# DigITs-AIML/MMNN_STS

Hardware: AMD Instinct MI355X
Metric: training volumes/sec/GPU (128^3 T1+T2+preop, batch 2) at 1/2/4/8 MI355X (higher is better)
Workload: dtype f32; 1 GPU; configs[2] --images --preop --survival --blend: MultiModalModel(DenseNet121-3D(in=2), MLP(32), blend) fwd + GradientBlender Cox loss + bwd + grad all-reduce + SGD-Nesterov/OneCycle step, dropout 0.2; micro_batch=2, global_batch=2, tabular=32, parallelism=dp1, allreduce=none

## Files before the change

mmnn_sts_amd/csrc/densenet.hip:

```cpp
#include "densenet.hpp"

#include <string.h>

#include <algorithm>

#include "fprop.hpp"
#include "stem.hpp"
#include "wgrad.hpp"

namespace mmnn {

constexpr size_t KZ_PART_BYTES = (size_t)512 * 4 * 1024 * sizeof(float);
constexpr unsigned KZ_CNT_ENTRIES = 4096;

namespace {
struct Panel { const float* p; unsigned bytes; };
struct LayerBind {
  BnFwd bn1, bn2;
  BnBwd gr_new, gr_t1;
  StatPtr dg1, dg2, s_x;
  View x, g;
  View x_new, g_new;
  View t1, dz2;
};
// ... 193 lines not shown
  return concat_site(p, b, lo.cin, lo.n1w, lo.n1b, lo.r1m, lo.r1v, p.o_dg_n1[b][l]);
}
static NormSite norm2(const Plan& p, int b, int l) {
  const LayerOff& lo = p.layers[b][l];
  return {p.o_st_t1[b][l], p.o_dg_n2[b][l], p.o_dg_n2[b][l], p.mid, 0, p.mid, p.nrep_b[b], lo.n2w, lo.n2b, lo.r2m, lo.r2v, (double)p.N * p.Vb[b]};
}
static NormSite transition(const Plan& p, int b) {
  const TransOff& t = p.trans[b];
  return concat_site(p, b, t.cin, t.nw, t.nb, t.rm, t.rv, p.o_dg_tr[b]);
}
static NormSite norm5(const Plan& p) {
  const int b = p.cfg.nblocks - 1;
  return concat_site(p, b, p.ctot_b[b], p.p_n5w, p.p_n5b, p.r_n5m, p.r_n5v, p.o_dg_n5);
}

static StatPtr statptr(char* ws, size_t o, int C, int off, int nrep) {
  StatPtr s; memset(&s, 0, sizeof(s));
  s.sum = reinterpret_cast<double*>(ws + o); s.sq = s.sum + (long)NREP * C;
  s.stride = C; s.off = off; s.nrep = nrep;
  return s;
}
static StatPtr stats(char* ws, const NormSite& s, int first = 0, int training = 1) {
  StatPtr st = statptr(ws, s.o_st, s.stride, s.off + first, s.nrep);
  if (!training) st.sum = nullptr;
  return st;
}
static StatPtr sums(char* ws, const NormSite& s, int first = 0) { return statptr(ws, s.o_s, s.stride, s.off + first, s.nrep); }
static StatPtr dgsums(char* ws, const NormSite& s) { return statptr(ws, s.o_dg, s.C, 0, s.nrep); }
static BnFwd bnfwd(const Plan& p, char* ws, const float* params, float* run, const NormSite& s, int training) {
  BnFwd f; memset(&f, 0, sizeof(f));
  f.st = stats(ws, s);
  f.rmean = run + s.rm; f.rvar = run + s.rv; f.gamma = params + s.w; f.beta = params + s.b;
  f.inv_count = 1.0 / s.count; f.eps = p.cfg.eps; f.training = training;
  return f;
}
static BnBwd bnbwd(const Plan& p, char* ws, const float* params, const NormSite& s, int first = 0) {
  BnBwd g; memset(&g, 0, sizeof(g));
  g.st = stats(ws, s, first); g.s = sums(ws, s, first);
  g.gamma = s.o_s == s.o_dg ? params + s.w : nullptr;
  g.inv_count = 1.0 / s.count; g.eps = p.cfg.eps;
  return g;
}

static float* fptr(char* ws, size_t o) { return reinterpret_cast<float*>(ws + o); }
static View concat(const Plan& p, char* ws, int b, int coff = 0) { return {fptr(ws, p.o_x[b]), (long)p.ctot_b[b] * p.Vb[b], coff}; }
static View concat_grad(const Plan& p, char* ws, int b, int coff = 0) { return {fptr(ws, p.o_g[b]), (long)p.ctot_b[b] * p.Vb[b], coff}; }
static View t1(const Plan& p, char* ws, int b, int l) { return {fptr(ws, p.o_t1[b][l]), (long)p.mid * p.Vb[b], 0}; }
static View dz2(const Plan& p, char* ws, int b, int l) { return {fptr(ws, p.o_dz2[b]) + (long)l * p.N * p.mid * p.Vb[b], (long)p.mid * p.Vb[b], 0}; }
static View pooled(const Plan& p, char* ws, int b) { return {fptr(ws, p.o_ap[b]), (long)p.ctot_b[b] * p.Vb[b + 1], 0}; }
static View pooled_grad(const Plan& p, char* ws, int b) { return {fptr(ws, p.o_dap), (long)p.ctot_b[b] * p.Vb[b + 1], 0}; }

static void set_in0(FpropArgs& a, View v) { a.in0 = v.p; a.in0_ns = v.ns; a.in0_coff = v.coff; }
static void set_in1(FpropArgs& a, View v) { a.in1 = v.p; a.in1_ns = v.ns; a.in1_coff = v.coff; }
static void set_out(FpropArgs& a, View v) { a.out = v.p; a.out_ns = v.ns; a.out_coff = v.coff; }
static void set_ex(FpropArgs& a, View v) { a.ex = v.p; a.ex_ns = v.ns; a.ex_coff = v.coff; }
static void set_g0(WgradArgs& a, View v) { a.g0 = v.p; a.g0_ns = v.ns; a.g0_coff = v.coff; }
static void set_g1(WgradArgs& a, View v) { a.g1 = v.p; a.g1_ns = v.ns; a.g1_coff = v.coff; }
static void set_x(WgradArgs& a, View v) { a.x = v.p; a.x_ns = v.ns; a.x_coff = v.coff; }

static Panel conv1_panel(const Plan& p, char* ws, int b, int l) { return {fptr(ws, p.o_pk_c1[b][l]), (unsigned)(sizeof(float) * conv1_elems(p, p.layers[b][l].cin))}; }
static Panel trans_panel(const Plan& p, char* ws, int b) { return {fptr(ws, p.o_pk_tr[b]), (unsigned)(sizeof(float) * trans_elems(p.trans[b]))}; }
static Panel conv1_weights(const Plan& p, const float* params, int b, int l) { return {params + p.layers[b][l].c1, (unsigned)(sizeof(float) * conv1_elems(p, p.layers[b][l].cin))}; }
static Panel conv2_panel(const Plan& p, char* ws, int b, int l, bool bwd, bool fp32 = false) {
  const size_t o3 = (bwd ? p.o_pk_c2b3 : p.o_pk_c2f3)[b][l];
  if (o3 && !fp32) return {fptr(ws, o3), (unsigned)conv2_split_bytes(p)};
  return {fptr(ws, (bwd ? p.o_pk_c2b : p.o_pk_c2f)[b][l]), (unsigned)(sizeof(float) * conv2_elems(p))};
}
static void set_conv2_weights(FpropArgs& a, const Plan& p, char* ws, int b, int l, bool bwd) {
  const Panel w = conv2_panel(p, ws, b, l, bwd, true), w3 = conv2_panel(p, ws, b, l, bwd);
  a.w = w.p;
  if (w3.p != w.p) { a.w3 = w3.p; a.x3 = ws + p.o_x3; a.x3_bytes = p.x3_bytes; }
}
static void prefetch(FpropArgs& a, Panel w) { a.pf_ptr = w.p; a.pf_bytes = w.bytes; }

static unsigned long long* trace_slot(const Plan& p) {
  return (p.trace_base && p.trace_seq < p.trace_slots) ? p.trace_base + (size_t)(p.trace_seq++) * 64 * 16 : nullptr;
}

static FpropArgs block_args(const Plan& p, char* ws, int b) {
  FpropArgs a; memset(&a, 0, sizeof(a));
  a.N = p.N; a.D = p.Db[b]; a.H = p.Hb[b]; a.W = p.Wb[b]; a.nrep = p.nrep_b[b];
  a.kz_part = p.no_kz ? nullptr : fptr(ws, p.o_kz_part); a.kz_cnt = reinterpret_cast<unsigned*>(ws + p.o_kz_cnt);
  a.kz_part_bytes = KZ_PART_BYTES; a.kz_cnt_entries = KZ_CNT_ENTRIES;
  a.trace = trace_slot(p);
  return a;
}
static void wgrad_shape(WgradArgs& w, const Plan& p, int b) {
  memset(&w, 0, sizeof(w));
  w.N = p.N; w.D = p.Db[b]; w.H = p.Hb[b]; w.W = p.Wb[b];
}

static bool build_tables(Plan& p, const float* params, float* run, char* ws) {
  if (p.tab_params == params && p.tab_run == run && p.tab_ws == ws) return false;
  char* hj = static_cast<char*>(p.host_jobs);
  RunStatJob* rj = reinterpret_cast<RunStatJob*>(hj);
  PackJob* pj = reinterpret_cast<PackJob*>(hj + (p.o_jobs_pack - p.o_jobs_run));
  GradJob* gj = reinterpret_cast<GradJob*>(hj + (p.o_jobs_grad - p.o_jobs_run));
  const NetCfg& c = p.cfg;
  const int nb = c.nblocks;
  int ir = 0, ip = 0, ig = 0;
  p.max_pack = 0; p.max_grad = 0;
  auto pack_job = [&](long src, size_t dst, int kind, int M, int C, long count) {
    PackJob& j = pj[ip++]; memset(&j, 0, sizeof(j));
    j.src = params + src; j.dst = fptr(ws, dst); j.kind = kind; j.M = M; j.C = C; j.count = count;
    p.max_pack = std::max(p.max_pack, count);
  };
  auto grad_job = [&](int kind, const void* src, long stride, int ns, int M, int C, long dst, long count) {
    GradJob& j = gj[ig++]; memset(&j, 0, sizeof(j));
    j.kind = kind; j.src = src; j.stride = stride; j.nsplit = ns; j.M = M; j.C = C; j.dst_off = dst; j.count = count;
    p.max_grad = std::max(p.max_grad, count);
  };
  auto grad_slab = [&](int kind, size_t o, int ns, int M, int C, long dst, long count) {
    grad_job(kind, ws + o, kind == 2 ? (long)C * M * 352 : count, ns, M, C, dst, count);
  };
  auto site_jobs = [&](const NormSite& s) {
    const StatPtr st = stats(ws, s), dg = dgsums(ws, s);
    RunStatJob& j = rj[ir++]; memset(&j, 0, sizeof(j));
    j.sum = st.sum; j.sq = st.sq; j.stride = s.stride; j.off = s.off; j.C = s.C;
    j.rmean = run ? run + s.rm : nullptr; j.rvar = run ? run + s.rv : nullptr; j.count = s.count;
    grad_job(3, dg.sq, s.C, 0, 0, s.C, s.w, s.C);
    grad_job(3, dg.sum, s.C, 0, 0, s.C, s.b, s.C);
  };
  pack_job(p.p_conv0, p.o_pk_conv0, (c.in_channels % 2 == 0) ? 3 : 4, c.init_features, c.in_channels, (long)7 * stem_krows(c.in_channels) * 64);
  grad_slab(2, p.o_sl_conv0, p.ns_conv0, c.init_features, c.in_channels, p.p_conv0, (long)c.init_features * c.in_channels * 343);
  site_jobs(norm0(p));
  for (int b = 0; b < nb; ++b) {
    p.gj_begin[b] = ig;
    const long max_before = p.max_grad;
    p.max_grad = 0;
    for (int l = 0; l < c.block_layers[b]; ++l) {
      const LayerOff& lo = p.layers[b][l];
      pack_job(lo.c1, p.o_pk_c1[b][l], 0, p.mid, lo.cin, conv1_elems(p, lo.cin));
      pack_job(lo.c2, p.o_pk_c2f[b][l], 1, c.growth, p.mid, conv2_elems(p));
      pack_job(lo.c2, p.o_pk_c2b[b][l], 2, c.growth, p.mid, conv2_elems(p));
      if (p.o_pk_c2f3[b][l]) pack_job(lo.c2, p.o_pk_c2f3[b][l], 5, c.growth, p.mid, (long)27 * (p.mid / 8) * c.growth);
      if (p.o_pk_c2b3[b][l]) pack_job(lo.c2, p.o_pk_c2b3[b][l], 6, c.growth, p.mid, (long)27 * (c.growth / 8) * p.mid);
      site_jobs(norm1(p, b, l));
      grad_slab(0, p.o_sl_c1[b][l], p.ns_c1[b][l], p.mid, lo.cin, lo.c1, conv1_elems(p, lo.cin));
      site_jobs(norm2(p, b, l));
      grad_slab(1, p.o_sl_c2[b][l], p.ns_c2[b][l], c.growth, p.mid, lo.c2, conv2_elems(p));
    }
    if (b != nb - 1) {
      const TransOff& t = p.trans[b];
      pack_job(t.cw, p.o_pk_tr[b], 0, t.cout, t.cin, trans_elems(t));
      site_jobs(transition(p, b));
      grad_slab(0, p.o_sl_tr[b], p.ns_tr[b], t.cout, t.cin, t.cw, trans_elems(t));
    } else {
      site_jobs(norm5(p));
    }
    p.gj_max[b] = p.max_grad;
    p.max_grad = std::max(p.max_grad, max_before);
  }
  p.gj_begin[nb] = ig;
  p.n_run_jobs = ir; p.n_pack_jobs = ip; p.n_grad_jobs = ig;
  p.tab_params = params; p.tab_run = run; p.tab_ws = ws;
  return true;
}

namespace {
struct ScopedTimer {
  Plan& p; hipStream_t s; bool on;
  ScopedTimer(Plan& p_, int kind, int block, hipStream_t s_) : p(p_), s(s_), on(false) {
    if (!((p.timer_mask >> kind) & 1u) || (p.timer_block >= 0 && p.timer_block != block)) return;
    if (p.timer_used + 2 > p.timer_ev.size()) {
      if (p.timer_ev.size() >= 16384) return;
      hipEvent_t a, b;
      if (hipEventCreate(&a) != hipSuccess || hipEventCreate(&b) != hipSuccess) return;
      p.timer_ev.push_back(a); p.timer_ev.push_back(b);
      p.timer_tag.push_back(0);
    }
    p.timer_tag[p.timer_used / 2] = kind * MAX_BLOCKS + (block >= 0 && block < MAX_BLOCKS ? block : 0);
    on = hipEventRecord(p.timer_ev[p.timer_used], s) == hipSuccess;
  }
  ~ScopedTimer() {
    if (!on) return;
    (void)hipEventRecord(p.timer_ev[p.timer_used + 1], s);
    p.timer_used += 2;
  }
};
}

int plan_set_timer(Plan& p, int kind, int block) {
  MMNN_REQUIRE(kind >= -1 && kind < T_COUNT, "set_timer: unknown kernel class %d", kind);
  p.timer_mask = kind < 0 ? ~1u : (kind == T_NONE ? 0u : 1u << kind);
  p.timer_block = block; p.timer_used = 0;
  for (int k = 0; k < T_COUNT * MAX_BLOCKS; ++k) { p.timer_ms[k] = 0.0; p.timer_count[k] = 0; }
  return 0;
}

int plan_read_timer(Plan& p, int kind, int block, double* total_ms, long* count) {
  MMNN_REQUIRE(kind >= T_NONE && kind < T_COUNT && block < MAX_BLOCKS, "read_timer: unknown kernel class %d / block %d", kind, block);
  for (size_t i = 0; i + 1 < p.timer_used; i += 2) {
    MMNN_HIP(hipEventSynchronize(p.timer_ev[i + 1]));
    float ms = 0.f;
    MMNN_HIP(hipEventElapsedTime(&ms, p.timer_ev[i], p.timer_ev[i + 1]));
    const int k = p.timer_tag[i / 2];
    p.timer_ms[k] += ms; p.timer_count[k] += 1;
  }
  p.timer_used = 0;
  double ms = 0.0; long n = 0;
  for (int k = 1; k < T_COUNT; ++k)
    for (int b = 0; b < MAX_BLOCKS; ++b)
      if ((kind == T_NONE || kind == k) && (block < 0 || block == b)) { ms += p.timer_ms[k * MAX_BLOCKS + b]; n += p.timer_count[k * MAX_BLOCKS + b]; }
  if (total_ms) *total_ms = ms;
  if (count) *count = n;
  return 0;
}

int plan_set_option(Plan& p, const char* name, long value) {
  const std::string s(name ? name : "");
  if (s == "single_stream") return 0;
  if (s == "trace_buffer") { p.trace_base = reinterpret_cast<unsigned long long*>(value); p.trace_seq = 0; return 0; }
  if (s == "trace_slots") { p.trace_slots = (int)value; return 0; }
  if (s == "params_version") { p.params_version = value; return 0; }
  if (s == "no_kz") { p.no_kz = value != 0; return 0; }
  set_error("set_option: unknown option '%s'", s.c_str());
  return 1;
}
static DropCfg dropcfg(const Plan& p, uint64_t seed, int layer, int training) {
  DropCfg d; memset(&d, 0, sizeof(d));
  d.seed = seed; d.layer = layer; d.p = training ? p.cfg.dropout_p : 0.f;
  return d;
}

int plan_forward(Plan& p, const float* params, float* run, const float* x, char* ws, float* out, int training, uint64_t seed,
                 hipStream_t stream) {
  MMNN_REQUIRE(params && run && x && ws && out, "forward: null buffer");
  MMNN_REQUIRE(((uintptr_t)ws & 255) == 0 && ((uintptr_t)params & 15) == 0 && ((uintptr_t)x & 15) == 0, "forward: buffers must be 256/16-byte aligned");
  const NetCfg& c = p.cfg;
  const int nb = c.nblocks, N = p.N;
  if (!p.host_jobs) {
    MMNN_HIP(hipHostMalloc(&p.host_jobs, p.host_jobs_bytes, hipHostMallocDefault));
    memset(p.host_jobs, 0, p.host_jobs_bytes);
  }
  if (p.tab_params != params || p.tab_run != run || p.tab_ws != ws) {
    if (p.tab_ws != nullptr) MMNN_HIP(hipStreamSynchronize(stream));
    build_tables(p, params, run, ws);
    MMNN_HIP(hipMemcpyAsync(ws + p.o_jobs_run, p.host_jobs, p.host_jobs_bytes, hipMemcpyHostToDevice, stream));
  }
  p.trace_seq = 0;
  if (training) MMNN_HIP(hipMemsetAsync(ws + p.o_fstat, 0, p.fstat_bytes, stream));
  MMNN_HIP(hipMemsetAsync(ws + p.o_kz_cnt, 0, KZ_CNT_ENTRIES * sizeof(unsigned), stream));
  int rc = 0;
  if (p.params_version == 0 || p.params_version != p.packed_version || p.packed_params != params || p.packed_ws != ws) {
    rc = launch_pack(reinterpret_cast<const PackJob*>(ws + p.o_jobs_pack), p.n_pack_jobs, p.max_pack, stream);
    if (rc) return rc;
    p.packed_version = p.params_version; p.packed_params = params; p.packed_ws = ws;
    ++p.pack_launches;
  }

  {
    const NormSite n0 = norm0(p);
    StemConvArgs a; memset(&a, 0, sizeof(a));
    a.N = N; a.Cin = c.in_channels; a.D = p.D; a.H = p.H; a.W = p.W; a.Do = p.D0; a.Ho = p.H0; a.Wo = p.W0; a.M = c.init_features;
    a.x = x; a.wp = fptr(ws, p.o_pk_conv0); a.out = fptr(ws, p.o_conv0);
    a.st_out = stats(ws, n0, 0, training);
    { ScopedTimer t(p, T_STEM_CONV, -1, stream); rc = launch_stem_conv(a, stream); }
    if (rc) return rc;
    const View X = concat(p, ws, 0);
    StemPoolArgs q; memset(&q, 0, sizeof(q));
    q.N = N; q.C = c.init_features; q.Di = p.D0; q.Hi = p.H0; q.Wi = p.W0; q.Do = p.Db[0]; q.Ho = p.Hb[0]; q.Wo = p.Wb[0];
    q.x = fptr(ws, p.o_conv0);
    q.bn = bnfwd(p, ws, params, run, n0, training);
    q.out = X.p; q.out_ns = X.ns;
    q.idx = reinterpret_cast<unsigned char*>(ws + p.o_idx);
    q.st_out = stats(ws, norm1(p, 0, 0), 0, training);
    if ((rc = launch_stem_pool(q, stream))) return rc;
  }
  int layer_id = 0;
  for (int b = 0; b < nb; ++b) {
    const View X = concat(p, ws, b);
    for (int l = 0; l < c.block_layers[b]; ++l, ++layer_id) {
      const NormSite n1 = norm1(p, b, l), n2 = norm2(p, b, l);
      FpropArgs a = block_args(p, ws, b);
      a.Cin = n1.C; a.M = p.mid;
      set_in0(a, X);
      a.bn_in = bnfwd(p, ws, params, run, n1, training);
      a.w = conv1_panel(p, ws, b, l).p; a.w_ld = p.mid;
      set_out(a, t1(p, ws, b, l));
      a.st_out = stats(ws, n2, 0, training);
      prefetch(a, conv2_panel(p, ws, b, l, false));
      { ScopedTimer t(p, T_CONV1_FWD, b, stream); rc = launch_fprop(a, 1, PRO_BNRELU, EPI_STORE_STATS, stream); }
      if (rc) return rc;
      FpropArgs e = block_args(p, ws, b);
      e.Cin = p.mid; e.M = c.growth;
      set_in0(e, t1(p, ws, b, l));
      e.bn_in = bnfwd(p, ws, params, run, n2, training);
      set_conv2_weights(e, p, ws, b, l, false); e.w_ld = c.growth;
      set_out(e, concat(p, ws, b, n1.C));
      e.drop_out = dropcfg(p, seed, layer_id, training);
      e.st_out = stats(ws, n1, n1.C, training);
      if (l + 1 < c.block_layers[b]) prefetch(e, conv1_panel(p, ws, b, l + 1));
      else if (b != nb - 1) prefetch(e, trans_panel(p, ws, b));
      { ScopedTimer t(p, T_CONV2_FWD, b, stream); rc = launch_fprop(e, 27, PRO_BNRELU, EPI_STORE_STATS, stream); }
      if (rc) return rc;
    }
    if (b != nb - 1) {
      const NormSite tr = transition(p, b);
// ... 186 lines not shown
      if ((rc = launch_wgrad1(w, PRO_NONE, stream))) return rc;
      FpropArgs d = block_args(p, ws, b);
      d.nrep = 0;
      d.Cin = t.cout; d.M = t.cin;
      set_in0(d, G); set_in1(d, X); d.gr_in = gr;
      d.w = params + t.cw; d.w_ld = t.cin;
      set_out(d, pooled_grad(p, ws, pb));
      if ((rc = launch_fprop(d, 1, PRO_GRAD, EPI_STORE, stream))) return rc;
      if ((rc = launch_consumer_bwd(consumer_bwd_args(p, params, run, ws, transition(p, pb), pb, 1, pooled_grad(p, ws, pb).p), stream))) return rc;
    } else {
      const NormSite n0 = norm0(p);
      const StatPtr dg = dgsums(ws, n0);
      StemPoolBwdArgs q; memset(&q, 0, sizeof(q));
      q.N = N; q.C = c.init_features; q.Di = p.D0; q.Hi = p.H0; q.Wi = p.W0; q.Do = p.Db[0]; q.Ho = p.Hb[0]; q.Wo = p.Wb[0];
      q.x = fptr(ws, p.o_conv0);
      q.bn = bnfwd(p, ws, params, run, n0, 1);
      q.g = G.p; q.g_ns = G.ns; q.xp = X.p; q.xp_ns = X.ns;
      q.gr = gr;
      q.idx = reinterpret_cast<const unsigned char*>(ws + p.o_idx);
      q.dz = fptr(ws, p.o_dz0);
      q.dbeta = dg.sum; q.dgamma = dg.sq;
      if ((rc = launch_stem_pool_bwd(q, stream))) return rc;
      StemWgradArgs w; memset(&w, 0, sizeof(w));
      w.N = N; w.Cin = c.in_channels; w.D = p.D; w.H = p.H; w.W = p.W; w.Do = p.D0; w.Ho = p.H0; w.Wo = p.W0; w.M = c.init_features;
      w.x = x; w.dz = fptr(ws, p.o_dz0); w.y = fptr(ws, p.o_conv0);
      w.gr = bnbwd(p, ws, params, n0);
      w.slab = fptr(ws, p.o_sl_conv0); w.slab_stride = (long)c.in_channels * c.init_features * 352; w.nsplit = p.ns_conv0;
      { ScopedTimer t(p, T_STEM_WGRAD, -1, stream); rc = launch_stem_wgrad(w, stream); }
      if (rc) return rc;
    }
  }
  const long stem_count = (long)c.init_features * c.in_channels * 343;
  const GradJob* jobs = reinterpret_cast<const GradJob*>(ws + p.o_jobs_grad);
  const int j0 = lo == 0 ? 0 : p.gj_begin[lo], j1 = p.gj_begin[hi + 1];
  long jmax = lo == 0 ? stem_count : 0;
  for (int b = lo; b <= hi; ++b) jmax = std::max(jmax, p.gj_max[b]);
  return launch_finalize(jobs + j0, j1 - j0, jmax, grad_params, accumulate, stream);
}

int plan_relu_mask(Plan& p, const float* params, char* ws, int kind, int b, int l, unsigned char* out, hipStream_t stream) {
  MMNN_REQUIRE(p.tab_ws == ws && p.tab_params == params, "relu_mask: must follow a training forward on the same buffers");
  const NetCfg& c = p.cfg;
  MMNN_REQUIRE(kind == 0 || (b >= 0 && b < c.nblocks), "relu_mask: bad block %d", b);
  MMNN_REQUIRE(kind != 3 || b < c.nblocks - 1, "relu_mask: block %d has no transition", b);
  MMNN_REQUIRE(kind == 0 || kind == 3 || (l >= 0 && l < c.block_layers[b] && (kind == 1 || kind == 2)), "relu_mask: bad site (%d,%d,%d)", kind, b, l);
  const NormSite s = kind == 0 ? norm0(p) : kind == 1 ? norm1(p, b, l) : kind == 2 ? norm2(p, b, l) : transition(p, b);
  const int V = kind == 0 ? p.D0 * p.H0 * p.W0 : p.Vb[b];
  const View X = kind == 0 ? View{fptr(ws, p.o_conv0), (long)s.C * V, 0} : kind == 2 ? t1(p, ws, b, l) : concat(p, ws, b);
  MaskArgs a; memset(&a, 0, sizeof(a));
  a.out = out; a.N = p.N; a.C = s.C; a.V = V; a.x = X.p; a.x_ns = X.ns;
  a.bn = bnfwd(p, ws, params, p.tab_run, s, 1);
  return launch_relu_mask(a, stream);
}

long plan_ws_offset(const Plan& p, const char* name, int i, int j) {
  const std::string s(name);
  const int nb = p.cfg.nblocks;
  auto okb = [&](int b) { return b >= 0 && b < nb; };
  auto okl = [&](int b, int l) { return okb(b) && l >= 0 && l < p.cfg.block_layers[b]; };
  if (s == "conv0") return (long)p.o_conv0;
  if (s == "idx") return (long)p.o_idx;
  if (s == "dz0") return (long)p.o_dz0;
  if (s == "dz2" && okl(i, j)) return (long)(p.o_dz2[i] + (size_t)j * p.N * p.mid * p.Vb[i] * sizeof(float));
  if (s == "dap") return (long)p.o_dap;
  if (s == "x" && okb(i)) return (long)p.o_x[i];
  if (s == "g" && okb(i)) return (long)p.o_g[i];
  if (s == "ap" && okb(i) && i < nb - 1) return (long)p.o_ap[i];
  if (s == "t1" && okl(i, j)) return (long)p.o_t1[i][j];
  if (s == "st_conv0") return (long)p.o_st_conv0;
  if (s == "st_x" && okb(i)) return (long)p.o_st_x[i];
  if (s == "st_t1" && okl(i, j)) return (long)p.o_st_t1[i][j];
  if (s == "s_x" && okb(i)) return (long)p.o_s_x[i];
  if (s == "pk_c1" && okl(i, j)) return (long)p.o_pk_c1[i][j];
  if (s == "pk_c2f" && okl(i, j)) return (long)p.o_pk_c2f[i][j];
  if (s == "pk_c2b" && okl(i, j)) return (long)p.o_pk_c2b[i][j];
  if (s == "pk_c2f3" && okl(i, j)) return p.o_pk_c2f3[i][j] ? (long)p.o_pk_c2f3[i][j] : -1;
  if (s == "pk_c2b3" && okl(i, j)) return p.o_pk_c2b3[i][j] ? (long)p.o_pk_c2b3[i][j] : -1;
  if (s == "x3") return p.x3_bytes ? (long)p.o_x3 : -1;
  if (s == "#x3_bytes") return (long)p.x3_bytes;
  if (s == "pk_conv0") return (long)p.o_pk_conv0;
  if (s == "#pack_launches") return p.pack_launches;
  if (s == "#ns_c2" && okl(i, j)) return p.ns_c2[i][j];
  if (s == "#ns_c1" && okl(i, j)) return p.ns_c1[i][j];
  return -1;
}

}
```

mmnn_sts_amd/csrc/densenet.hpp:

```cpp
#pragma once
#include <string>
#include <vector>

#include "common.hpp"
#include "elementwise.hpp"

namespace mmnn {

constexpr int MAX_BLOCKS = 8;

struct NetCfg {
  int in_channels, init_features, growth, bn_size, nblocks;
  int block_layers[MAX_BLOCKS];
  float eps, momentum, dropout_p;
};

struct LayerOff {
  long n1w, n1b, c1, n2w, n2b, c2;
  long r1m, r1v, r2m, r2v;
  int cin;
};
struct TransOff { long nw, nb, cw; long rm, rv; int cin, cout; };

struct NormSite {
  size_t o_st;
  size_t o_s;
  size_t o_dg;
  int stride, off, C, nrep;
  long w, b, rm, rv;
  double count;
};
struct View { float* p; long ns; int coff; };

struct Plan {
  NetCfg cfg;
  int N, D, H, W;
  int D0, H0, W0;
  int Db[MAX_BLOCKS], Hb[MAX_BLOCKS], Wb[MAX_BLOCKS], Vb[MAX_BLOCKS];
  int cin_b[MAX_BLOCKS], ctot_b[MAX_BLOCKS];
  int nrep_b[MAX_BLOCKS];
  int mid;
  long p_conv0, p_n0w, p_n0b, r_n0m, r_n0v, p_n5w, p_n5b, r_n5m, r_n5v;
  std::vector<std::vector<LayerOff>> layers;
  std::vector<TransOff> trans;
  long n_params, n_runstats;
  int n_bn;
  size_t ws_bytes;
  size_t o_conv0, o_idx, o_x[MAX_BLOCKS], o_g[MAX_BLOCKS], o_ap[MAX_BLOCKS], o_dz2[MAX_BLOCKS], o_dap, o_dz0;
  std::vector<std::vector<size_t>> o_t1;
  size_t o_fstat, fstat_bytes, o_bstat, bstat_bytes;
  size_t o_st_conv0, o_st_x[MAX_BLOCKS];
  std::vector<std::vector<size_t>> o_st_t1;
  size_t o_s_x[MAX_BLOCKS];
  size_t o_dg_n0, o_dg_n5;
  std::vector<std::vector<size_t>> o_dg_n1, o_dg_n2;
  std::vector<size_t> o_dg_tr;
  size_t o_pk_conv0;
  std::vector<std::vector<size_t>> o_pk_c1, o_pk_c2f, o_pk_c2b;
  std::vector<std::vector<size_t>> o_pk_c2f3, o_pk_c2b3;
  size_t o_x3 = 0, x3_bytes = 0;
  std::vector<size_t> o_pk_tr;
  size_t o_sl_conv0; int ns_conv0;
  std::vector<std::vector<size_t>> o_sl_c1, o_sl_c2;
  std::vector<std::vector<int>> ns_c1, ns_c2;
  std::vector<size_t> o_sl_tr; std::vector<int> ns_tr;
  size_t o_kz_part, o_kz_cnt;
  size_t o_jobs_run, o_jobs_pack, o_jobs_grad;
  int n_layers = 0;
  size_t o_wg_table = 0;
  void* wg_pinned = nullptr; std::vector<char> wg_shadow; bool wg_uploaded = false;
  void* host_jobs = nullptr; size_t host_jobs_bytes = 0;
  const float* tab_params = nullptr; float* tab_run = nullptr; char* tab_ws = nullptr;
  int n_run_jobs = 0, n_pack_jobs = 0, n_grad_jobs = 0; long max_pack = 0, max_grad = 0;
  int gj_begin[MAX_BLOCKS + 1] = {0};
  long gj_max[MAX_BLOCKS] = {0};
  unsigned timer_mask = 0; int timer_block = -1;
  std::vector<hipEvent_t> timer_ev;
  std::vector<int> timer_tag;
  size_t timer_used = 0;
  double timer_ms[16 * MAX_BLOCKS] = {0}; long timer_count[16 * MAX_BLOCKS] = {0};
  long params_version = 0, packed_version = 0; const float* packed_params = nullptr; const char* packed_ws = nullptr;
  long pack_launches = 0;
  long long* nbt = nullptr; int nbt_count = 0;
  bool no_kz = false;
  int bwd_next = -1;
  unsigned long long* trace_base = nullptr; mutable int trace_seq = 0; int trace_slots = 0;
};

enum TimerKind { T_NONE = 0, T_CONV2_FWD = 1, T_CONV2_DGRAD = 2, T_CONV2_WGRAD = 3, T_CONV1_FWD = 4, T_CONV1_DGRAD = 5,
                 T_CONV1_WGRAD = 6, T_STEM_CONV = 7, T_STEM_WGRAD = 8, T_BLOCK_FWD = 9, T_COUNT = 10 };
int plan_set_timer(Plan& p, int kind, int block);
int plan_read_timer(Plan& p, int kind, int block, double* total_ms, long* count);
int plan_set_option(Plan& p, const char* name, long value);

int plan_build(Plan& p, const NetCfg& cfg, int N, int D, int H, int W);
void plan_free(Plan& p);
int plan_forward(Plan& p, const float* params, float* runstats, const float* x, char* ws, float* out, int training,
                 uint64_t seed, hipStream_t stream);
int plan_backward(Plan& p, const float* params, const float* x, char* ws, const float* grad_out, float* grad_params,
                  int accumulate, uint64_t seed, hipStream_t stream);
int plan_backward_range(Plan& p, const float* params, const float* x, char* ws, const float* grad_out, float* grad_params,
                        int accumulate, uint64_t seed, int hi, int lo, hipStream_t stream);
int plan_block_param_range(const Plan& p, int block, long* begin, long* end);
long plan_ws_offset(const Plan& p, const char* name, int i, int j);
int plan_relu_mask(Plan& p, const float* params, char* ws, int kind, int b, int l, unsigned char* out, hipStream_t stream);

}
```

mmnn_sts_amd/csrc/fprop.hip:

```cpp
#include <stdlib.h>

#include "fprop.hpp"

namespace mmnn {

template <int TAPS, int PRO, int EPI>
int dispatch(const FpropArgs& a, hipStream_t s);
extern template int dispatch<1, PRO_BNRELU, EPI_STORE_STATS>(const FpropArgs&, hipStream_t);
extern template int dispatch<1, PRO_NONE, EPI_STORE_STATS>(const FpropArgs&, hipStream_t);
extern template int dispatch<1, PRO_GRAD, EPI_MASK_ACCUM>(const FpropArgs&, hipStream_t);
extern template int dispatch<1, PRO_GRAD, EPI_STORE>(const FpropArgs&, hipStream_t);
extern template int dispatch<27, PRO_BNRELU, EPI_STORE_STATS>(const FpropArgs&, hipStream_t);
extern template int dispatch<27, PRO_GRAD, EPI_MASK_STORE>(const FpropArgs&, hipStream_t);

bool conv3_fwd_bf16x3_eligible(const FpropArgs& a);
int launch_conv3_fwd_bf16x3(const FpropArgs& a, hipStream_t stream);
bool conv3_dgrad_bf16x3_eligible(const FpropArgs& a);
int launch_conv3_dgrad_bf16x3(const FpropArgs& a, hipStream_t stream);

int launch_fprop(const FpropArgs& a, int taps, int pro, int epi, hipStream_t stream) {
  MMNN_REQUIRE(a.N > 0 && a.D > 0 && a.H > 0 && a.W > 0 && a.Cin > 0 && a.M > 0, "fprop: non-positive extent");
  MMNN_REQUIRE((long)a.D * a.H * a.W < (1l << 30), "fprop: volume too large for 32-bit voxel indices");
  MMNN_REQUIRE(a.in0 && a.w && a.out && a.w_ld >= a.M, "fprop: null operand or w_ld < M");
  MMNN_REQUIRE((long)(a.M + 128) * a.D * a.H * a.W < (1l << 31), "fprop: output rows x volume too large for 32-bit element offsets");
  MMNN_REQUIRE(pro != PRO_GRAD || a.in1, "fprop: PRO_GRAD needs the normalised tensor (in1)");
  MMNN_REQUIRE((epi != EPI_MASK_STORE && epi != EPI_MASK_ACCUM) || (a.ex && a.dgamma && a.dbeta), "fprop: mask epilogue operands missing");
  if (taps == 27 && pro == PRO_BNRELU && epi == EPI_STORE_STATS && conv3_fwd_bf16x3_eligible(a)) return launch_conv3_fwd_bf16x3(a, stream);
  if (taps == 27 && pro == PRO_GRAD && epi == EPI_MASK_STORE && conv3_dgrad_bf16x3_eligible(a)) return launch_conv3_dgrad_bf16x3(a, stream);
#define MMNN_CASE(T, P, E) \
  if (taps == T && pro == P && epi == E) return dispatch<T, P, E>(a, stream);
  MMNN_CASE(1, PRO_BNRELU, EPI_STORE_STATS)
  MMNN_CASE(1, PRO_NONE, EPI_STORE_STATS)
  MMNN_CASE(1, PRO_GRAD, EPI_MASK_ACCUM)
  MMNN_CASE(1, PRO_GRAD, EPI_STORE)
  MMNN_CASE(27, PRO_BNRELU, EPI_STORE_STATS)
  MMNN_CASE(27, PRO_GRAD, EPI_MASK_STORE)
#undef MMNN_CASE
  set_error("fprop: unsupported (taps=%d, pro=%d, epi=%d)", taps, pro, epi);
  return 1;
}

}
```

mmnn_sts_amd/csrc/fprop.hpp:

```cpp
#pragma once
#include "common.hpp"

namespace mmnn {

#if !defined(MMNN_KZ_FENCED)
#if defined(__gfx950__) || !defined(__HIP_DEVICE_COMPILE__)
#define MMNN_KZ_FENCED 0
#else
#define MMNN_KZ_FENCED 1
#endif
#endif

enum Pro { PRO_NONE = 0, PRO_BNRELU = 1, PRO_GRAD = 2 };
enum Epi { EPI_STORE = 0, EPI_STORE_STATS = 1, EPI_MASK_STORE = 2, EPI_MASK_ACCUM = 3 };

struct FpropArgs {
  int N, D, H, W;
  int Cin, M;
  const float* in0; long in0_ns; int in0_coff;
  const float* in1; long in1_ns; int in1_coff;
  BnFwd bn_in;
  BnBwd gr_in;
  DropCfg drop_in;
  const float* w; int w_ld;
  float* out; long out_ns; int out_coff;
  DropCfg drop_out;
  StatPtr st_out;
  const float* ex; long ex_ns; int ex_coff;
  BnFwd ebn;
  double* dgamma; double* dbeta;
  StatPtr s_acc;
  int nrep;
  float* kz_part; unsigned* kz_cnt;
  size_t kz_part_bytes; unsigned kz_cnt_entries;
  const float* pf_ptr; unsigned pf_bytes;
  const void* w3; void* x3; size_t x3_bytes;
  unsigned mg_w, mg_h, mg_d;
  unsigned long long* trace;
};

int launch_fprop(const FpropArgs& a, int taps, int pro, int epi, hipStream_t stream);
bool conv3_fwd_bf16x3_eligible(const FpropArgs& a);
bool conv3_dgrad_bf16x3_eligible(const FpropArgs& a);
size_t conv3_bf16x3_plane_bytes(const FpropArgs& a);

#if defined(__HIPCC__)

template <int TAPS, int PRO, int EPI, int WM, int WN, int KS, int MT, int NT, int KC, int TD, int TH, int TW, bool SPEC = false>
struct FpropCfg {
  static constexpr int NWAVES = WM * WN * KS;
  static constexpr int NCOMPUTE = NWAVES * 64;
  static constexpr int NTHREADS = NCOMPUTE * (SPEC ? 2 : 1);
  static constexpr int M_B = WM * MT * 32;
  static constexpr int V_B = WN * NT * 32;
  static constexpr int RS = (TAPS == 27) ? TW + 8 : TW;
  static constexpr int HS = (TAPS == 27) ? TH + 2 : 1;
  static constexpr int DS = (TAPS == 27) ? TD + 2 : 1;
  static constexpr int XS = DS * HS * RS;
  static constexpr int NCOEF = (PRO == PRO_BNRELU) ? 2 : (PRO == PRO_GRAD ? 3 : 0);
  static constexpr int ECOEF = 6 + 2 * WN;
  static_assert(TD * TH * TW == V_B, "tile volume must equal the block's voxel count");
  static_assert(KC % 2 == 0 && (KC / 2) % KS == 0, "channel-pair count of a chunk must be a multiple of the K-split");
  static constexpr int STAGE = KC * XS + KC * TAPS * M_B;
  static constexpr bool DIST = (MT * NT == 1) && KS > 1 && !SPEC;
  static constexpr int REDN = (DIST ? KS : KS - 1) * WM * WN * MT * NT * 1024;
  static constexpr int BUF0 = ((SPEC ? 2 : 1) * STAGE) > REDN ? ((SPEC ? 2 : 1) * STAGE) : REDN;
  static constexpr bool WIDE = (EPI == EPI_MASK_STORE || EPI == EPI_MASK_ACCUM || (EPI == EPI_STORE_STATS && !(TAPS == 27 && WM * WN > 1))) && !SPEC;
  static constexpr int TSTRIDE = 36;
  static constexpr int TRANS = WIDE ? WM * WN * 32 * TSTRIDE : 0;
  static constexpr int BUF = BUF0 > TRANS ? BUF0 : TRANS;
  static size_t smem_bytes(int Cin) {
    int cpad = ((Cin + KC - 1) / KC) * KC;
    size_t ncoef = ((size_t)NCOEF * cpad + 3) & ~(size_t)3;
    return sizeof(float) * (ncoef + (size_t)BUF + (size_t)ECOEF * M_B + 4);
  }
};

template <int PRO>
__device__ __forceinline__ float pro_apply(const float* coef, int cpad, int c, float x0, float x1) {
  if (PRO == PRO_BNRELU) return fmaxf(fmaf(coef[c], x0, coef[cpad + c]), 0.f);
  if (PRO == PRO_GRAD) return fmaf(coef[c], x0, fmaf(coef[cpad + c], x1, coef[2 * cpad + c]));
  return x0;
}

template <int R>
__device__ __forceinline__ float half_reduce_n(const float (&v)[R], int lane) {
  static_assert(R == 2 || R == 4 || R == 8, "half_reduce_n: 2, 4 or 8 registers");
  float w[R];
#pragma unroll
  for (int r = 0; r < R; ++r) w[r] = v[r];
  if (R >= 8) {
    const bool b = lane & 16;
#pragma unroll
    for (int r = 0; r < 4; ++r) { const float send = b ? w[r] : w[r + 4], keep = b ? w[r + 4] : w[r]; w[r] = keep + swz_xor<16>(send); }
  }
  if (R >= 4) {
    constexpr int X = (R == 8) ? 8 : 16;
    const bool b = lane & X;
#pragma unroll
    for (int r = 0; r < 2; ++r) { const float send = b ? w[r] : w[r + 2], keep = b ? w[r + 2] : w[r]; w[r] = keep + swz_xor<X>(send); }
  }
  {
    constexpr int X = (R == 8) ? 4 : (R == 4 ? 8 : 16);
    const bool b = lane & X;
    const float send = b ? w[0] : w[1], keep = b ? w[1] : w[0];
    w[0] = keep + swz_xor<X>(send);
  }
  float t = w[0];
  if (R <= 2) t += swz_xor<8>(t);
  if (R <= 4) t += swz_xor<4>(t);
  t += swz_xor<2>(t);
  t += swz_xor<1>(t);
  return t;
}

template <int TAPS, int PRO, int EPI, int WM, int WN, int KS, int MT, int NT, int KC, int TD, int TH, int TW, bool SPEC = false>
__global__ void __launch_bounds__(WM* WN* KS * 64 * (SPEC ? 2 : 1)) fprop_kernel(const FpropArgs a) {
  using C = FpropCfg<TAPS, PRO, EPI, WM, WN, KS, MT, NT, KC, TD, TH, TW, SPEC>;
  constexpr int NL = C::NCOMPUTE;
  constexpr int NTHREADS = C::NTHREADS, M_B = C::M_B, V_B = C::V_B, RS = C::RS, HS = C::HS, DS = C::DS, XS = C::XS;
  extern __shared__ __attribute__((aligned(16))) float smem[];
  const int tid = threadIdx.x, lane = tid & 63;
#if defined(MMNN_PHASE_TRACE)
  const bool tracing = a.trace != nullptr && tid == 0 && blockIdx.x < 64 && blockIdx.y == 0;
#else
  constexpr bool tracing = false;
#endif
// ... 1052 lines not shown
```

Before: 260.2 volumes/s (whole job; 1 volume = 1 patient = stacked T1+T2 2x128^3 + 32 tabular).

## Add resident-operand 1x1x1 conv dgrad kernel with mask-accumulate epilogue

```diff
diff --git a/mmnn_sts_amd/csrc/conv1_dgrad.hip b/mmnn_sts_amd/csrc/conv1_dgrad.hip
--- /dev/null
+++ b/mmnn_sts_amd/csrc/conv1_dgrad.hip
@@ -0,0 +1,338 @@
+#include <algorithm>
+
+#include "fprop.hpp"
+
+namespace mmnn {
+
+namespace {
+constexpr int RK = 128;
+constexpr int RVT = 64;
+constexpr int RMS = 64;
+constexpr int RKC = 64;
+constexpr int RTHREADS = 256;
+constexpr int RTS = 36;
+constexpr int R_COEF = 3 * RK, R_Z = RK * RVT, R_W = RKC * RMS, R_T = 4 * 32 * RTS, R_E = 2 * 5 * RMS, R_RED = 2 * 2 * RMS;
+constexpr size_t R_SMEM = sizeof(float) * (R_COEF + R_Z + R_W + R_T + R_E + R_RED);
+constexpr int R_FILL = 512;
+}
+
+#if defined(__HIPCC__)
+template <int KS>
+__global__ void __launch_bounds__(RTHREADS, 2) conv1_dgrad_resident_kernel(const FpropArgs a) {
+  static_assert(KS == 1 || KS == 2 || KS == 8, "conv1_dgrad_resident: K-split of a fprop_kernel 1x1x1 tile");
+  constexpr int GPC = KS > 1 ? KS / 2 : 1, NPG = (RKC / 2) / GPC;
+  auto pair_of = [](int h, int lp) { return KS == 1 ? h * (RKC / 2) + lp : h * GPC + lp / NPG + (lp % NPG) * KS; };
+  extern __shared__ __attribute__((aligned(16))) float smem[];
+  float* coef = smem;
+  float* Zs = coef + R_COEF;
+  float* Ws = Zs + R_Z;
+  float* Tb = Ws + R_W;
+  float* ecoef = Tb + R_T;
+  float* red = ecoef + R_E;
+  const int tid = threadIdx.x, lane = tid & 63, wave = tid >> 6, half = lane >> 5, l31 = lane & 31;
+  const int wm = wave >> 1, wn = wave & 1;
+  kernarg_warm<sizeof(FpropArgs)>();
+  const int V = a.D * a.H * a.W, M = a.M;
+  const int nt = (V + RVT - 1) / RVT;
+  const int n = (int)blockIdx.x / nt, v0 = ((int)blockIdx.x - n * nt) * RVT;
+  const int nsteps = (M + RMS - 1) / RMS;
+  const int t_begin = (nsteps * (int)blockIdx.y) / (int)gridDim.y, t_end = (nsteps * ((int)blockIdx.y + 1)) / (int)gridDim.y;
+  const int rep = blockIdx.x & ((a.nrep > 0 ? a.nrep : NREP) - 1);
+  const float* in0n = a.in0 + (long)n * a.in0_ns + (long)a.in0_coff * V;
+  const float* in1n = a.in1 + (long)n * a.in1_ns + (long)a.in1_coff * V;
+  const float* exn = a.ex + (long)n * a.ex_ns + (long)a.ex_coff * V;
+  float* outn = a.out + (long)n * a.out_ns + (long)a.out_coff * V;
+  const int q4 = 4 * (lane & 7), rl = lane >> 3;
+  const int vq = v0 + wn * 32 + q4;
+
+  const bool fast_gr = a.gr_in.st.nrep <= 2 && a.gr_in.s.nrep <= 2;
+  const bool fast_e = a.ebn.training && a.ebn.st.nrep <= 2;
+  BnBwdRaw raw_gr;
+  BnFwdRaw raw_e;
+  if (tid < RK && fast_gr) bn_bwd_issue(a.gr_in, tid, raw_gr);
+
+  f32x4 wreg[4];
+  auto load_w = [&](int t, int h) {
+#pragma unroll
+    for (int i = 0; i < 4; ++i) {
+      const int it = tid + i * RTHREADS, q = it & 15, kr = it >> 4;
+      const bool ok = t < t_end && t * RMS + 4 * q < M;
+      wreg[i] = *reinterpret_cast<const f32x4*>(ok ? a.w + (long)(2 * pair_of(h, kr >> 1) + (kr & 1)) * a.w_ld + t * RMS + 4 * q : a.w);
+    }
+  };
+  auto store_w = [&](int t) {
+#pragma unroll
+    for (int i = 0; i < 4; ++i) {
+      const int it = tid + i * RTHREADS, q = it & 15;
+      const bool ok = t * RMS + 4 * q < M;
+      *reinterpret_cast<f32x4*>(Ws + 4 * it) = ok ? wreg[i] : f32x4{0.f, 0.f, 0.f, 0.f};
+    }
+  };
+  f32x4 xqA[4], gqA[4], xqB[4], gqB[4];
+  auto load_xg = [&](int t, f32x4 (&xq)[4], f32x4 (&gq)[4]) {
+#pragma unroll
+    for (int k = 0; k < 4; ++k) {
+      const int m = t * RMS + wm * 32 + rl + 8 * k;
+      const unsigned off = (t < t_end && m < M && vq < V) ? (unsigned)m * (unsigned)V + (unsigned)vq : 0u;
+      xq[k] = *reinterpret_cast<const f32x4*>(exn + off);
+      gq[k] = *reinterpret_cast<const f32x4*>(outn + off);
+    }
+  };
+  auto ecoef_issue = [&](int t) {
+    if (tid < RMS && fast_e) bn_fwd_issue(a.ebn, min(t * RMS + tid, M - 1), raw_e);
+  };
+  auto ecoef_finish = [&](int t) {
+    if (tid < RMS) {
+      const int m = t * RMS + tid;
+      float ea = 0.f, eb = 0.f, mu = 0.f, rs = 0.f, g = 0.f;
+      if (fast_e) {
+        bn_fwd_finish(a.ebn, raw_e, ea, eb, mu, rs);
+        g = raw_e.g;
+      } else if (m < M) {
+        bn_fwd_coef(a.ebn, m, ea, eb, mu, rs);
+        g = a.ebn.gamma[m];
+      }
+      if (m >= M) { ea = 0.f; eb = 0.f; mu = 0.f; rs = 0.f; g = 0.f; }
+      float* e = ecoef + (t & 1) * (5 * RMS);
+      e[tid] = ea; e[RMS + tid] = eb; e[2 * RMS + tid] = mu; e[3 * RMS + tid] = rs; e[4 * RMS + tid] = g;
+    }
+  };
+
+  load_w(t_begin, 0);
+  f32x4 z0[8], z1[8];
+#pragma unroll
+  for (int i = 0; i < 8; ++i) {
+    const int it = tid + i * RTHREADS, q = it & 15, k = it >> 4;
+    const int off = (v0 + 4 * q < V) ? k * V + v0 + 4 * q : 0;
+    z0[i] = *reinterpret_cast<const f32x4*>(in0n + off);
+    z1[i] = *reinterpret_cast<const f32x4*>(in1n + off);
+  }
+  ecoef_issue(t_begin);
+  if (tid < RK) {
+    float p = 0.f, q = 0.f, r = 0.f;
+    if (fast_gr) bn_bwd_finish(a.gr_in, raw_gr, p, q, r);
+    else bn_bwd_coef(a.gr_in, tid, p, q, r);
+    const float sc = drop_scale(a.drop_in, n, tid);
+    coef[tid] = p * sc; coef[RK + tid] = q * sc; coef[2 * RK + tid] = r * sc;
+  }
+  __syncthreads();
+#pragma unroll
+  for (int i = 0; i < 8; ++i) {
+    const int it = tid + i * RTHREADS, q = it & 15, k = it >> 4;
+    f32x4 o;
+#pragma unroll
+    for (int e = 0; e < 4; ++e) o[e] = pro_apply<PRO_GRAD>(coef, RK, k, z0[i][e], z1[i][e]);
+    if (!(v0 + 4 * q < V)) o = f32x4{0.f, 0.f, 0.f, 0.f};
+    *reinterpret_cast<f32x4*>(Zs + 4 * it) = o;
+  }
+  ecoef_finish(t_begin);
+  store_w(t_begin);
+  load_xg(t_begin, xqA, gqA);
+  float pf_sink = 0.f, pf_sink2 = 0.f;
+  {
+    const unsigned lines = a.pf_bytes >> 7;
+    if (a.pf_ptr != nullptr && lines != 0) {
+      const unsigned lin = blockIdx.x + gridDim.x * blockIdx.y;
+      const unsigned per_xcd = (gridDim.x * gridDim.y + 7u) >> 3;
+      const unsigned ln0 = (lin >> 3) * RTHREADS + tid, ln1 = ln0 + per_xcd * RTHREADS;
+      pf_sink = a.pf_ptr[(size_t)min(ln0, lines - 1) * 32];
+      pf_sink2 = a.pf_ptr[(size_t)min(ln1, lines - 1) * 32];
+    }
+  }
+
+  f32x16 acc, partA, partB;
+  auto mfma_chunk = [&](int h) {
+    const float* zb = Zs + half * RVT + wn * 32 + l31;
+    const float* wb = Ws + half * RMS + wm * 32 + l31;
+    const f32x16 zero = {0.f, 0.f, 0.f, 0.f, 0.f, 0.f, 0.f, 0.f, 0.f, 0.f, 0.f, 0.f, 0.f, 0.f, 0.f, 0.f};
+    auto fold = [&](int g, const f32x16& p) {
+      if (h == 0 && g == 0) acc = p;
+      else acc += p;
+    };
+    auto mm = [&](int lp, float av, float bv) {
+      if constexpr (KS == 1) {
+        acc = __builtin_amdgcn_mfma_f32_32x32x2f32(av, bv, acc, 0, 0, 0);
+      } else {
+        const int g = lp / NPG, j = lp % NPG;
+        if (g & 1) partB = __builtin_amdgcn_mfma_f32_32x32x2f32(av, bv, j == 0 ? zero : partB, 0, 0, 0);
+        else partA = __builtin_amdgcn_mfma_f32_32x32x2f32(av, bv, j == 0 ? zero : partA, 0, 0, 0);
+        if (g > 0 && j == 1) fold(g - 1, (g & 1) ? partA : partB);
+        if (g == GPC - 1 && j == NPG - 1) fold(g, (g & 1) ? partB : partA);
+      }
+    };
+    float a0, b0, a1, b1;
+    a0 = wb[0]; b0 = zb[pair_of(h, 0) * 2 * RVT];
+#pragma unroll
+    for (int s = 0; s < RKC / 2; s += 2) {
+      a1 = wb[(s + 1) * 2 * RMS]; b1 = zb[pair_of(h, s + 1) * 2 * RVT];
+      __builtin_amdgcn_sched_group_barrier(0x100, 2, 0);
+      mm(s, a0, b0);
+      __builtin_amdgcn_sched_group_barrier(0x008, 1, 0);
+      if (s + 2 < RKC / 2) { a0 = wb[(s + 2) * 2 * RMS]; b0 = zb[pair_of(h, s + 2) * 2 * RVT]; }
+      __builtin_amdgcn_sched_group_barrier(0x100, 2, 0);
+      mm(s + 1, a1, b1);
+      __builtin_amdgcn_sched_group_barrier(0x008, 1, 0);
+    }
+  };
+  auto flush_sums = [&](int t) {
+    const int m = t * RMS + tid;
+    if (tid < RMS && m < M) {
+      double v0d = 0.0, v1d = 0.0;
+#pragma unroll
+      for (int j = 0; j < 2; ++j) { v0d += (double)red[j * RMS + tid]; v1d += (double)red[2 * RMS + j * RMS + tid]; }
+      atomicAdd(a.dbeta + (long)rep * M + m, v0d);
+      atomicAdd(a.dgamma + (long)rep * M + m, v1d);
+      const double g = (double)ecoef[(t & 1) * (5 * RMS) + 4 * RMS + tid];
+      atomicAdd(a.s_acc.sum + (long)rep * a.s_acc.stride + a.s_acc.off + m, g * v0d);
+      atomicAdd(a.s_acc.sq + (long)rep * a.s_acc.stride + a.s_acc.off + m, g * v1d);
+    }
+  };
+
+  auto step = [&](int t, f32x4 (&xq)[4], f32x4 (&gq)[4], f32x4 (&xn)[4], f32x4 (&gn)[4]) {
+    if constexpr (KS == 1) {
+#pragma unroll
+      for (int r = 0; r < 16; ++r) acc[r] = 0.f;
+    }
+    __syncthreads();
+    if (t > t_begin) flush_sums(t - 1);
+    if (t + 1 < t_end) ecoef_issue(t + 1);
+    load_w(t, 1);
+    load_xg(t + 1, xn, gn);
+    mfma_chunk(0);
+    if (t + 1 < t_end) ecoef_finish(t + 1);
+    __syncthreads();
+    store_w(t);
+    __syncthreads();
+    load_w(t + 1, 0);
+    mfma_chunk(1);
+    __syncthreads();
+    const float* e = ecoef + (t & 1) * (5 * RMS);
+    float* tb = Tb + wave * (32 * RTS);
+    __builtin_amdgcn_fence(__ATOMIC_ACQ_REL, "wavefront");
+    __builtin_amdgcn_wave_barrier();
+#pragma unroll
+    for (int r = 0; r < 16; ++r) tb[acc_row(r, half) * RTS + l31] = acc[r];
+    __builtin_amdgcn_fence(__ATOMIC_ACQ_REL, "wavefront");
+    __builtin_amdgcn_wave_barrier();
+    f32x4 o[4];
+    unsigned off[4];
+    bool ok[4];
+    float zs[4][4], xhs[4][4];
+#pragma unroll
+    for (int k = 0; k < 4; ++k) {
+      const int ml = wm * 32 + rl + 8 * k, m = t * RMS + ml;
+      const f32x4 vt = *reinterpret_cast<const f32x4*>(tb + (rl + 8 * k) * RTS + q4);
+      ok[k] = m < M && vq < V;
+      off[k] = ok[k] ? (unsigned)m * (unsigned)V + (unsigned)vq : 0u;
+      const float ea = e[ml], eb = e[RMS + ml], mu = e[2 * RMS + ml], rs = e[3 * RMS + ml], gm = e[4 * RMS + ml];
+#pragma unroll
+      for (int c = 0; c < 4; ++c) {
+        const float x = xq[k][c];
+        const float pre = fmaf(ea, x, eb);
+        const float z = (ok[k] && pre > 0.f) ? vt[c] : 0.f;
+        zs[k][c] = z;
+        xhs[k][c] = ok[k] ? (x - mu) * rs : 0.f;
+        o[k][c] = gq[k][c] + gm * z;
+      }
+      if constexpr (KS > 1) {
+        float s0[4], s1[4];
+#pragma unroll
+        for (int c = 0; c < 4; ++c) {
+          s0[c] = zs[k][c]; s1[c] = zs[k][c] * xhs[k][c];
+          s0[c] += swz_xor<4>(s0[c]); s1[c] += swz_xor<4>(s1[c]);
+          s0[c] += swz_xor<2>(s0[c]); s1[c] += swz_xor<2>(s1[c]);
+          s0[c] += swz_xor<1>(s0[c]); s1[c] += swz_xor<1>(s1[c]);
+        }
+        const float t0 = (s0[0] + s0[2]) + (s0[1] + s0[3]), t1 = (s1[0] + s1[2]) + (s1[1] + s1[3]);
+        if ((lane & 7) == 0) {
+          red[wn * RMS + ml] = t0;
+          red[2 * RMS + wn * RMS + ml] = t1;
+        }
+      }
+    }
+    if constexpr (KS == 1) {
+      float* xb = Tb + (wm * 2) * (32 * RTS);
+      __syncthreads();
+      if (wn == 1) {
+#pragma unroll
+        for (int k = 0; k < 4; ++k)
+#pragma unroll
+          for (int c = 0; c < 4; ++c) { xb[((k * 4 + c) * 2) * 64 + lane] = zs[k][c]; xb[((k * 4 + c) * 2 + 1) * 64 + lane] = xhs[k][c]; }
+      }
+      __syncthreads();
+#pragma unroll
+      for (int k = 0; k < 4; ++k) {
+        const int ml = wm * 32 + rl + 8 * k;
+        float t0 = 0.f, t1 = 0.f;
+        if (wn == 0) {
+#pragma unroll
+          for (int c = 0; c < 4; ++c) { t0 += zs[k][c]; t1 += zs[k][c] * xhs[k][c]; }
+#pragma unroll
+          for (int c = 0; c < 4; ++c) {
+            const float z = xb[((k * 4 + c) * 2) * 64 + lane], xh = xb[((k * 4 + c) * 2 + 1) * 64 + lane];
+            t0 += z; t1 += z * xh;
+          }
+          t0 += swz_xor<1>(t0); t1 += swz_xor<1>(t1);
+          t0 += swz_xor<2>(t0); t1 += swz_xor<2>(t1);
+          t0 += swz_xor<4>(t0); t1 += swz_xor<4>(t1);
+        }
+        if ((lane & 7) == 0) {
+          red[wn * RMS + ml] = t0;
+          red[2 * RMS + wn * RMS + ml] = t1;
+        }
+      }
+    }
+    store_w(t + 1);
+#pragma unroll
+    for (int k = 0; k < 4; ++k)
+      if (ok[k]) *reinterpret_cast<f32x4*>(outn + off[k]) = o[k];
+  };
+  for (int t = t_begin; t < t_end; t += 2) {
+    step(t, xqA, gqA, xqB, gqB);
+    if (t + 1 < t_end) step(t + 1, xqB, gqB, xqA, gqA);
+  }
+  __syncthreads();
+  flush_sums(t_end - 1);
+  if (pf_sink + pf_sink2 == 1.2345678e-33f) a.out[0] = pf_sink;
+}
+#endif
+
+bool conv1_dgrad_resident_shape_ok(int mode, int N, long V, int Cin, int M, int w_ld) {
+  if (mode == 0 || N <= 0 || V <= 0) return false;
+  if (Cin != RK || (V & 3) != 0 || (M & 3) != 0 || (w_ld & 3) != 0 || (long)(M + RK) * V >= (1l << 31)) return false;
+  if ((long)N * cdiv(V, RVT) >= (1l << 31) / RTHREADS) return false;
+  if (mode == 1 && (V < 512 || (long)N * cdiv(V, RVT) > R_FILL)) return false;
+  return true;
+}
+
+bool conv1_dgrad_resident_eligible(const FpropArgs& a) {
+  const long V = (long)a.D * a.H * a.W;
+  if (!conv1_dgrad_resident_shape_ok(a.conv1_dgrad_resident, a.N, V, a.Cin, a.M, a.w_ld)) return false;
+  if (!a.in0 || !a.in1 || !a.ex || !a.out || !a.w || !a.dgamma || !a.dbeta || !a.s_acc.sum || !a.s_acc.sq) return false;
+  const uintptr_t ptrs = (uintptr_t)a.in0 | (uintptr_t)a.in1 | (uintptr_t)a.ex | (uintptr_t)a.out | (uintptr_t)a.w;
+  const long strides = a.in0_ns | a.in1_ns | a.ex_ns | a.out_ns;
+  return (ptrs & 15) == 0 && (strides & 3) == 0;
+}
+
+template <int KS>
+static int launch_ks(const FpropArgs& a, dim3 grid, hipStream_t stream) {
+  if (int rc = allow_dynamic_lds<conv1_dgrad_resident_kernel<KS>>(R_SMEM)) return rc;
+  MMNN_LAUNCH(conv1_dgrad_resident_kernel<KS>, grid, dim3(RTHREADS), R_SMEM, stream, a);
+  MMNN_HIP(hipGetLastError());
+  return 0;
+}
+
+int launch_conv1_dgrad_resident(const FpropArgs& a, hipStream_t stream) {
+  MMNN_REQUIRE(conv1_dgrad_resident_eligible(a), "conv1_dgrad_resident: shape not eligible");
+  const long V = (long)a.D * a.H * a.W;
+  const long tiles = (long)a.N * cdiv(V, RVT);
+  const int nsteps = cdiv(a.M, RMS);
+  const int rg = (int)std::min<long>(nsteps, std::max<long>(1, R_FILL / tiles));
+  const long blocks_a = (long)a.N * cdiv(V, 128) * cdiv(a.M, 128), blocks_b = (long)a.N * cdiv(V, 64) * cdiv(a.M, 64);
+  const dim3 grid((unsigned)tiles, (unsigned)rg);
+  if (blocks_a >= 192) return launch_ks<1>(a, grid, stream);
+  if (blocks_b >= 192) return launch_ks<2>(a, grid, stream);
+  return launch_ks<8>(a, grid, stream);
+}
+
+}
diff --git a/mmnn_sts_amd/csrc/densenet.hip b/mmnn_sts_amd/csrc/densenet.hip
--- a/mmnn_sts_amd/csrc/densenet.hip
+++ b/mmnn_sts_amd/csrc/densenet.hip
@@ -299,6 +299,7 @@
   a.N = p.N; a.D = p.Db[b]; a.H = p.Hb[b]; a.W = p.Wb[b]; a.nrep = p.nrep_b[b];
   a.kz_part = p.no_kz ? nullptr : fptr(ws, p.o_kz_part); a.kz_cnt = reinterpret_cast<unsigned*>(ws + p.o_kz_cnt);
   a.kz_part_bytes = KZ_PART_BYTES; a.kz_cnt_entries = KZ_CNT_ENTRIES;
+  a.conv1_dgrad_resident = p.conv1_dgrad_resident;
   a.trace = trace_slot(p);
   return a;
 }
@@ -431,6 +432,11 @@
   if (s == "trace_slots") { p.trace_slots = (int)value; return 0; }
   if (s == "params_version") { p.params_version = value; return 0; }
   if (s == "no_kz") { p.no_kz = value != 0; return 0; }
+  if (s == "conv1_dgrad_resident") {
+    MMNN_REQUIRE(value >= 0 && value <= 2, "set_option: conv1_dgrad_resident is 0, 1 or 2");
+    p.conv1_dgrad_resident = (int)value;
+    return 0;
+  }
   set_error("set_option: unknown option '%s'", s.c_str());
   return 1;
 }
@@ -783,6 +789,12 @@
   if (s == "#pack_launches") return p.pack_launches;
   if (s == "#ns_c2" && okl(i, j)) return p.ns_c2[i][j];
   if (s == "#ns_c1" && okl(i, j)) return p.ns_c1[i][j];
+  if (s == "#conv1_dgrad_resident" && okb(i)) {
+    long cnt = 0;
+    for (int l = 0; l < p.cfg.block_layers[i]; ++l)
+      cnt += conv1_dgrad_resident_shape_ok(p.conv1_dgrad_resident, p.N, p.Vb[i], p.mid, p.layers[i][l].cin, p.layers[i][l].cin) ? 1 : 0;
+    return cnt;
+  }
   return -1;
 }
 
diff --git a/mmnn_sts_amd/csrc/densenet.hpp b/mmnn_sts_amd/csrc/densenet.hpp
--- a/mmnn_sts_amd/csrc/densenet.hpp
+++ b/mmnn_sts_amd/csrc/densenet.hpp
@@ -82,6 +82,7 @@
   long params_version = 0, packed_version = 0; const float* packed_params = nullptr; const char* packed_ws = nullptr;
   long pack_launches = 0;
   long long* nbt = nullptr; int nbt_count = 0;
+  int conv1_dgrad_resident = 1;
   bool no_kz = false;
   int bwd_next = -1;
   unsigned long long* trace_base = nullptr; mutable int trace_seq = 0; int trace_slots = 0;
diff --git a/mmnn_sts_amd/csrc/fprop.hip b/mmnn_sts_amd/csrc/fprop.hip
--- a/mmnn_sts_amd/csrc/fprop.hip
+++ b/mmnn_sts_amd/csrc/fprop.hip
@@ -27,6 +27,7 @@
   MMNN_REQUIRE((epi != EPI_MASK_STORE && epi != EPI_MASK_ACCUM) || (a.ex && a.dgamma && a.dbeta), "fprop: mask epilogue operands missing");
   if (taps == 27 && pro == PRO_BNRELU && epi == EPI_STORE_STATS && conv3_fwd_bf16x3_eligible(a)) return launch_conv3_fwd_bf16x3(a, stream);
   if (taps == 27 && pro == PRO_GRAD && epi == EPI_MASK_STORE && conv3_dgrad_bf16x3_eligible(a)) return launch_conv3_dgrad_bf16x3(a, stream);
+  if (taps == 1 && pro == PRO_GRAD && epi == EPI_MASK_ACCUM && conv1_dgrad_resident_eligible(a)) return launch_conv1_dgrad_resident(a, stream);
 #define MMNN_CASE(T, P, E) \
   if (taps == T && pro == P && epi == E) return dispatch<T, P, E>(a, stream);
   MMNN_CASE(1, PRO_BNRELU, EPI_STORE_STATS)
diff --git a/mmnn_sts_amd/csrc/fprop.hpp b/mmnn_sts_amd/csrc/fprop.hpp
--- a/mmnn_sts_amd/csrc/fprop.hpp
+++ b/mmnn_sts_amd/csrc/fprop.hpp
@@ -31,6 +31,7 @@
   double* dgamma; double* dbeta;
   StatPtr s_acc;
   int nrep;
+  int conv1_dgrad_resident;
   float* kz_part; unsigned* kz_cnt;
   size_t kz_part_bytes; unsigned kz_cnt_entries;
   const float* pf_ptr; unsigned pf_bytes;
@@ -43,6 +44,9 @@
 bool conv3_fwd_bf16x3_eligible(const FpropArgs& a);
 bool conv3_dgrad_bf16x3_eligible(const FpropArgs& a);
 size_t conv3_bf16x3_plane_bytes(const FpropArgs& a);
+bool conv1_dgrad_resident_shape_ok(int mode, int N, long V, int Cin, int M, int w_ld);
+bool conv1_dgrad_resident_eligible(const FpropArgs& a);
+int launch_conv1_dgrad_resident(const FpropArgs& a, hipStream_t stream);
 
 #if defined(__HIPCC__)
 
```

After: 264.5 volumes/s (whole job; 1 volume = 1 patient = stacked T1+T2 2x128^3 + 32 tabular) (median of 6 runs). 1.02x the previous value.
